# ruiminshen/yolo2-pytorch

Hardware: NVIDIA H100
Metric: 416x416 images/sec (higher is better)
Workload: dtype f16

## Files before the change

include/yolo2_b200.h:

```cpp
#ifndef YOLO2_B200_H_
#define YOLO2_B200_H_

#ifdef __cplusplus
extern "C" {
#endif

typedef void* yb_stream_t;

#define YB_ERR_BAD_ARG (-1)
#define YB_ERR_UNSUPPORTED (-2)
#define YB_ERR_DRIVER (-3)

#define YB_OUT_F16_NHWC 0
#define YB_OUT_F32_NCHW 1
#define YB_CONV_A_TILED 1
#define YB_CONV_WIDE_N 2
#define YB_CONV_FORCE_BN(bn) ((bn) << 8)
#define YB_CONV_POOL2X2 16
#define YB_CONV_C32_IM2COL 32
#define YB_CONV_NO_STREAMK 8
#define YB_CONV_FORCE_STREAMK (1 << 30)
#define YB_CONV_NO_SMALLK (1 << 28)
#define YB_CONV_PLAIN_STORE (1 << 29)
#define YB_FILTER_THRESHOLD 0
#define YB_FILTER_FIX 1
#define YB_FILTER_NONE 2

int yb_version(void);
const char* yb_last_error(void);
int yb_debug_read(int out[4]);
int yb_conv_set_trace(void* dev_buf);

int yb_pack_weight_f16(const float* w_oihw, void* w_f16, int cout, int cin, int ksize, int mode, yb_stream_t stream);
int yb_bn_fold(const float* gamma, const float* beta, const float* running_mean, const float* running_var, float eps, float* scale,
               float* shift, int channels, yb_stream_t stream);

int yb_conv0_bn_leaky_pool_fwd(const float* x_nchw, const float* w_oihw, const float* scale, const float* shift, float slope,
                               void* y_nhwc_f16, int batch, int height, int width, int cout, yb_stream_t stream);
int yb_conv0_u8_bn_leaky_pool_fwd(const unsigned char* x_nhwc_u8, const float* w_oihw, const float* scale, const float* shift,
                                  float slope, void* y_nhwc_f16, int batch, int height, int width, int cout, yb_stream_t stream);
int yb_conv_bn_act_fwd(const void* x, const void* w, const float* scale, const float* shift, float slope, void* y, int batch,
                       int height, int width, int cin, int cout, int ksize, int x_ld, long long y_ld, int y_ch_off, int out_mode,
                       int flags, yb_stream_t stream);
int yb_conv_bn_act_stats_fwd(const void* x, const void* w, const float* scale, const float* shift, float slope, void* y, int batch,
                             int height, int width, int cin, int cout, int ksize, int x_ld, long long y_ld, int y_ch_off, int flags,
                             double* sums, yb_stream_t stream);
long long yb_conv_workspace_bytes(void);
int yb_conv_choice(int batch, int height, int width, int cin, int cout, int ksize, int out_mode, int flags, int with_workspace, int out[6]);
int yb_conv_bn_act_fwd_ws(const void* x, const void* w, const float* scale, const float* shift, float slope, void* y, int batch,
                          int height, int width, int cin, int cout, int ksize, int x_ld, long long y_ld, int y_ch_off, int out_mode,
                          int flags, void* workspace, long long workspace_bytes, yb_stream_t stream);
int yb_conv_bn_act_split_fwd(const void* x, const void* w_split, const float* scale, const float* shift, float slope, void* y, int batch,
// ... 140 lines not shown
```

yolo2-pytorch_b200/b200/ops.py:

```python
import ctypes

import torch

from . import lib as _l

OUT_F16_NHWC, OUT_F32_NCHW = 0, 1
CONV_A_TILED, CONV_WIDE_N = 1, 2
CONV_NO_STREAMK, CONV_FORCE_STREAMK, CONV_NO_SMALLK, CONV_PLAIN_STORE = 8, 1 << 30, 1 << 28, 1 << 29
CONV_POOL2X2, CONV_C32_IM2COL, CONV_C32_SWAP = 16, 32, 64
FILTER_THRESHOLD, FILTER_FIX, FILTER_NONE = 0, 1, 2


launch_count = 0


def _ck(rc, what):
    global launch_count
    _l.check(rc, what)
    launch_count += 1


def conv_force_bn(bn):
    return bn << 8


def conv_force_mt(mt):
    return mt << 20


def conv_force_pair(v):
    return v << 22


CONV_ALLOW_PAIR = 4


def _p(t):
    return None if t is None else ctypes.c_void_p(t.data_ptr())


def _s():
    return ctypes.c_void_p(torch.cuda.current_stream().cuda_stream)
# ... 57 lines not shown
def conv0_u8_bn_leaky_pool(x, w, scale, shift, slope, out=None):
    _req(x, torch.uint8, 'x'); _req(w, torch.float32, 'w'); _req(scale, torch.float32, 'scale'); _req(shift, torch.float32, 'shift')
    b, h, wd, c = x.shape
    if c != 3:
        raise ValueError('conv0 expects 3 input channels')
    cout = w.shape[0]
    if out is None:
        out = torch.empty(b, h // 2, wd // 2, cout, dtype=torch.float16, device=x.device)
    _req(out, torch.float16, 'out')
    _ck(_l.load().yb_conv0_u8_bn_leaky_pool_fwd(_p(x), _p(w), _p(scale), _p(shift), float(slope), _p(out), b, h, wd, cout, _s()),
        'yb_conv0_u8_bn_leaky_pool_fwd')
    return out


def _conv_common(fn_name, x, w, scale, shift, slope, out, batch, height, width, cin, cout, k, x_ld, y_ld, y_ch_off, out_mode, flags,
                 workspace=None):
    if workspace is not None and fn_name == 'yb_conv_bn_act_fwd':
        fn_name = 'yb_conv_bn_act_fwd_ws'
    fn = getattr(_l.load(), fn_name)
    args = [_p(x), _p(w), _p(scale), _p(shift), float(slope), _p(out), batch, height, width, cin, cout, k, x_ld, y_ld, y_ch_off, out_mode]
    if fn_name != 'yb_conv_ref_fwd':
        args.append(flags)
    if fn_name == 'yb_conv_bn_act_fwd_ws':
        _req(workspace, torch.uint8, 'workspace')
        args += [_p(workspace), workspace.numel()]
    args.append(_s())
    _ck(fn(*args), fn_name)


def conv_workspace(device='cuda'):
    return torch.zeros(int(_l.load().yb_conv_workspace_bytes()), dtype=torch.uint8, device=device)


CONV_KERNELS = ('conv_igemm_kernel', 'conv_wide_kernel', 'conv_c32_kernel')


def conv_choice(batch, height, width, cin, cout, k, out_mode=OUT_F16_NHWC, flags=0, workspace=True):
    out = (ctypes.c_int * 6)()
    _l.check(_l.load().yb_conv_choice(batch, height, width, cin, cout, k, out_mode, flags, int(bool(workspace)), ctypes.byref(out)),
             'yb_conv_choice')
    return dict(kernel=CONV_KERNELS[out[0]], bk=out[1], bn=out[2], rows=out[3], streamk=bool(out[4]), grid=out[5])


def conv_bn_act(x, w, scale, shift, slope, out=None, out_mode=OUT_F16_NHWC, y_ch_off=0, cin=None, flags=0, ref=False, workspace=None):
    _req(x, torch.float16, 'x'); _req(w, torch.float16, 'w'); _req(scale, torch.float32, 'scale'); _req(shift, torch.float32, 'shift')
    b, h, wd, x_ld = x.shape
    cout, k, _, wcin = w.shape
    cin = wcin if cin is None else cin
    if cin != wcin:
        raise ValueError('weight Cin %d != %d' % (wcin, cin))
    if out is None:
        oh, ow = (h // 2, wd // 2) if (flags & CONV_POOL2X2) else (h, wd)
        out = (torch.empty(b, oh, ow, cout, dtype=torch.float16, device=x.device) if out_mode == OUT_F16_NHWC
               else torch.empty(b, cout, h, wd, dtype=torch.float32, device=x.device))
    if out_mode == OUT_F16_NHWC:
        _req(out, torch.float16, 'out')
        y_ld = out.shape[-1]
    else:
        _req(out, torch.float32, 'out')
        y_ld = 0
    _conv_common('yb_conv_ref_fwd' if ref else 'yb_conv_bn_act_fwd', x, w, scale, shift, slope, out, b, h, wd, cin, cout, k, x_ld, y_ld,
                 y_ch_off, out_mode, flags, workspace=None if ref else workspace)
    return out


def conv1x1_preact(x, w, pre_scale, pre_shift, pre_relu, scale, shift, slope, out=None, out_mode=OUT_F16_NHWC, y_ch_off=0, cin=None, flags=0,
                   workspace=None):
# ... 216 lines not shown
```

yolo2-pytorch_b200/csrc/conv_igemm.cu:

```cuda
#include "yb_common.h"
#include "yb_ptx.cuh"
#include <stdlib.h>

namespace yb {

struct ConvParams {
  int m_total;
  int height, width;
  int cin, cout;
  int ksize, pad;
  int kb_per_tap;
  int num_kb;
  int m_tiles, n_tiles;
  int a_im2col;
  const float* scale;
  const float* shift;
  float slope;
  void* y;
  long long y_ld;
  int y_ch_off;
  int out_mode;
  int hw;
  int skip;
  int* dbg;
// ... 739 lines not shown
          for (int h = 0; h < 2; ++h) {
#pragma unroll
            for (int hh = 0; hh < 2; ++hh) {
              const int j = c2 * 8 + jj;
              float x0 = acc[h][4 * j + 2 * hh] * sc0 + sh0;
              float x1 = acc[h][4 * j + 2 * hh + 1] * sc1 + sh1;
              x0 = x0 > 0.f ? x0 : x0 * p.slope;
              x1 = x1 > 0.f ? x1 : x1 * p.slope;
              __half2 v = __floats2half2_rn(x0, x1);
              const int r = h * 64 + warp * 16 + (lane >> 2) + hh * 8;
              const uint32_t addr = stage_o + r * 128 + ((jj ^ (r & 7)) << 4) + 4 * (lane & 3);
              asm volatile("st.shared.b32 [%0], %1;" :: "r"(addr), "r"(*reinterpret_cast<uint32_t*>(&v)) : "memory");
            }
          }
        }
        fence_proxy_async_smem();
        asm volatile("bar.sync %0, 128;" :: "r"(2 + cw) : "memory");
        if (t == 0) {
#pragma unroll
          for (int g = 0; g < 4; ++g)
            if (m_base + 32 * g < p.m_total) tma_store_2d(&tmap_y, stage_o + g * 4096, n0 + c2 * 64, m_base + 32 * g);
          tma_store_commit();
        }
      }
    }
    if (sk_collect) {
      asm volatile("bar.sync 1, 256;" ::: "memory");
      for (int j = sk_lo + t + 128 * cw; j < static_cast<int>(blockIdx.x); j += 256) p.flags[j] = 0u;
    }
  }
  if (t == 0) tma_store_wait<0>();
}

struct C32Params {
  int batch, height, width, cout;
  int tiles_w, tiles_h, num_tiles;
  const float* scale;
  const float* shift;
  float slope;
  int pool;
  int swap_lbo;
  int skip;
  int* dbg;
  unsigned long long* trace;
  double* stats;
};

struct C32Cfg {
  static constexpr int TH = 16, TW = 8, HH = TH + 2, HW = TW + 2;
  static constexpr int kPlaneData = HH * HW * 16;
  static constexpr int kPlane = (kPlaneData + 127) / 128 * 128;
  static constexpr int kHalo = 4 * kPlane;
  static constexpr int kStages = 4;
  static constexpr int BN = 64;
  static constexpr int kBTap = BN * 32 * 2;
  static constexpr int kBBytes = 9 * kBTap;
  static constexpr int kOutBytes = 128 * 128;
  static constexpr int kGroups = 2;
  static constexpr int kAccBytes = BN * kAccPitch * 4;
  static constexpr int kEpiThreads = kGroups * 128;
  static constexpr int kThreads = 128 + 32 + kEpiThreads;
  static constexpr int kSmemBytes = 1024 + kBBytes + 2 * kGroups * kOutBytes + kStages * kHalo + kGroups * kAccBytes + 2 * BN * 4 + 256 + 2 * BN * 4 ;
  static_assert(kSmemBytes <= kSmemLimit, "c32: shared memory budget");
};

__global__ void __launch_bounds__(C32Cfg::kThreads, 1)
// ... 186 lines not shown
      asm volatile("bar.sync %0, 128;" :: "r"(1 + grp) : "memory");
      if (et == 0) { YB_TRACE(2, tr); ++tr; }
      if (writer) {
#pragma unroll
        for (int c = 0; c < 8; ++c) st_shared_v4(obuf + srow * 128 + ((c ^ (srow & 7)) << 4), pk[c]);
      }
      fence_proxy_async_smem();
      asm volatile("bar.sync %0, 128;" :: "r"(1 + grp) : "memory");
      if (gt == 0 && !(p.skip & 8)) {
        if (p.pool) tma_store_4d(&tmap_y, obuf, 0, tw * (Cfg::TW / 2), th * (Cfg::TH / 2), n);
        else tma_store_4d(&tmap_y, obuf, 0, tw * Cfg::TW, th * Cfg::TH, n);
        tma_store_commit();
      }
      if (et == 0) { YB_TRACE(2, tr); ++tr; }
    }
    if (gt == 0) tma_store_wait<0>();
    if (p.stats != nullptr) {
      asm volatile("bar.sync 8, %0;" :: "n"(Cfg::kEpiThreads) : "memory");
      for (int i = et; i < p.cout; i += Cfg::kEpiThreads) {
        atomicAdd(p.stats + i, static_cast<double>(ep_stats[i]));
        atomicAdd(p.stats + p.cout + i, static_cast<double>(ep_stats[BN + i]));
      }
    }
  }
}

constexpr long long kSkFlagBytes = 4096;
constexpr long long kSkSlotBytes = kWideRows * kWideBN * 4;
long long conv_workspace_bytes() { return kSkFlagBytes + kSkSlotBytes * sm_count(); }

constexpr int kKernelIgemm = 0;
constexpr int kKernelWide = 1;
constexpr int kKernelC32 = 2;
struct ConvChoice {
  int kernel, bk, bn, mt, streamk, grid;
};

static unsigned long long* g_conv_trace = nullptr;
void conv_set_trace(void* dev_ptr) { g_conv_trace = static_cast<unsigned long long*>(dev_ptr); }

typedef CUresult (*EncodeTiledFn)(CUtensorMap*, CUtensorMapDataType, cuuint32_t, void*, const cuuint64_t*, const cuuint64_t*,
                                  const cuuint32_t*, const cuuint32_t*, CUtensorMapInterleave, CUtensorMapSwizzle,
                                  CUtensorMapL2promotion, CUtensorMapFloatOOBfill);
typedef CUresult (*EncodeIm2colFn)(CUtensorMap*, CUtensorMapDataType, cuuint32_t, void*, const cuuint64_t*, const cuuint64_t*,
                                   const int*, const int*, cuuint32_t, cuuint32_t, const cuuint32_t*, CUtensorMapInterleave,
                                   CUtensorMapSwizzle, CUtensorMapL2promotion, CUtensorMapFloatOOBfill);

static int get_encoders(EncodeTiledFn* tiled, EncodeIm2colFn* im2col) {
  static EncodeTiledFn s_tiled = nullptr;
  static EncodeIm2colFn s_im2col = nullptr;
  if (s_tiled == nullptr || s_im2col == nullptr) {
    void* f0 = nullptr;
    void* f1 = nullptr;
    cudaDriverEntryPointQueryResult q0, q1;
    YB_CUDA(cudaGetDriverEntryPoint("cuTensorMapEncodeTiled", &f0, cudaEnableDefault, &q0));
    YB_CUDA(cudaGetDriverEntryPoint("cuTensorMapEncodeIm2col", &f1, cudaEnableDefault, &q1));
    if (f0 == nullptr || f1 == nullptr || q0 != cudaDriverEntryPointSuccess || q1 != cudaDriverEntryPointSuccess)
      return fail(YB_ERR_DRIVER, "cuTensorMapEncode* driver entry points unavailable");
    s_tiled = reinterpret_cast<EncodeTiledFn>(f0);
    s_im2col = reinterpret_cast<EncodeIm2colFn>(f1);
  }
  *tiled = s_tiled;
  *im2col = s_im2col;
  return 0;
}

int get_tensor_map_encoders(EncodeTiledFn* tiled, EncodeIm2colFn* im2col) { return get_encoders(tiled, im2col); }

// ... 31 lines not shown
  if (pre != nullptr) {
    YB_CUDA(cudaLaunchKernelEx(&cfg, conv_preact_kernel<BN, BK, MT>, ta, tb, ty, p, *pre));
    return check_launch("conv_preact_kernel");
  }
  YB_CUDA(cudaLaunchKernelEx(&cfg, conv_igemm_kernel<BN, BK, MT>, ta, tb, ty, p));
  return check_launch("conv_igemm_kernel");
}

template <int BK>
static int launch_wide(const CUtensorMap& ta, const CUtensorMap& tb, const CUtensorMap& ty, const ConvParams& p, int grid, cudaStream_t stream) {
  using Cfg = WideCfg<BK>;
  static bool attr_set = false;
  if (!attr_set) {
    YB_CUDA(cudaFuncSetAttribute(conv_wide_kernel<BK>, cudaFuncAttributeMaxDynamicSharedMemorySize, Cfg::kSmemBytes));
    attr_set = true;
  }
  cudaLaunchConfig_t cfg;
  memset(&cfg, 0, sizeof(cfg));
  cudaLaunchAttribute attr[1];
  int nattr = 0;
  static const int use_pdl = getenv("YB_PDL") ? atoi(getenv("YB_PDL")) : 0;
  if (use_pdl) {
    attr[nattr].id = cudaLaunchAttributeProgrammaticStreamSerialization;
    attr[nattr].val.programmaticStreamSerializationAllowed = 1;
    ++nattr;
  }
  cfg.gridDim = dim3(grid);
  cfg.blockDim = dim3(kWideThreads);
  cfg.dynamicSmemBytes = Cfg::kSmemBytes;
  cfg.stream = stream;
  cfg.attrs = attr; cfg.numAttrs = nattr;
  YB_CUDA(cudaLaunchKernelEx(&cfg, conv_wide_kernel<BK>, ta, tb, ty, p));
  return check_launch("conv_wide_kernel");
}

template <int BK>
static int dispatch_conv(int bn, int mt, int grid, const CUtensorMap& ta, const CUtensorMap& tb, const CUtensorMap& ty, const ConvParams& p,
                         const PreAct* pre, cudaStream_t stream) {
  if (mt == 2 && bn == 128) return launch_wide<BK>(ta, tb, ty, p, grid, stream);
  if (mt == 2) return launch_conv<64, BK, 2>(ta, tb, ty, p, pre, stream);
  if (bn == 64) return launch_conv<64, BK, 1>(ta, tb, ty, p, pre, stream);
  return launch_conv<128, BK, 1>(ta, tb, ty, p, pre, stream);
}

static int conv_c32_forward(const void* x, const void* w, const float* scale, const float* shift, float slope, void* y, int batch,
                            int height, int width, int cout, int x_ld, long long y_ld, int y_ch_off, int pool, int flags, double* stats,
                            cudaStream_t stream) {
  using Cfg = C32Cfg;
  EncodeTiledFn enc_tiled;
  EncodeIm2colFn enc_im2col;
  int rc = get_encoders(&enc_tiled, &enc_im2col);
  if (rc) return rc;
  YB_REQUIRE(!pool || (height % 2 == 0 && width % 2 == 0), "conv: fused 2x2 max-pool needs even H and W");
  C32Params p;
  p.batch = batch; p.height = height; p.width = width; p.cout = cout;
  p.tiles_w = (width + Cfg::TW - 1) / Cfg::TW;
  p.tiles_h = (height + Cfg::TH - 1) / Cfg::TH;
  const long long nt = static_cast<long long>(batch) * p.tiles_w * p.tiles_h;
  YB_REQUIRE(nt < (1ll << 31), "conv: too many tiles");
  p.num_tiles = static_cast<int>(nt);
  p.scale = scale; p.shift = shift; p.slope = slope;
  p.pool = pool;
  p.swap_lbo = (flags >> 6) & 1;
  p.skip = (flags >> 24) & 0xF;
  p.dbg = debug_word_device();
  p.trace = g_conv_trace;
// ... 43 lines not shown

constexpr double kKbNsIm2col = 240.0;
constexpr double kKbNsTiled = 100.0;
constexpr double kFeedBytesPerNs = 130.0;
constexpr double kEpiNsPerOut = 0.15;
constexpr double kWideEpiNsPerOut = 0.08;
constexpr double kSkNs = 16000.0;
constexpr double kSkNsWide = 9000.0;
int conv_choose(int batch, int height, int width, int cin, int cout, int ksize, int a_channels, int out_mode, int flags, bool workspace_ok,
                bool stats, bool lo, bool pre, ConvChoice* out) {
  ConvChoice c;
  memset(&c, 0, sizeof(c));
  const int sms = sm_count();
  const bool split = a_channels != cin || lo;
  if (!split && cin == 32 && ksize == 3 && cout <= 64 && out_mode == 0 && ((flags >> 28) & 1) == 0 && ((flags >> 5) & 1) == 0 && ((flags >> 8) & 0xFFFF) == 0) {
    const long long tiles = static_cast<long long>(batch) * ((width + C32Cfg::TW - 1) / C32Cfg::TW) * ((height + C32Cfg::TH - 1) / C32Cfg::TH);
    c.kernel = kKernelC32; c.bk = 32; c.bn = C32Cfg::BN; c.mt = 1;
    c.grid = static_cast<int>(tiles < sms ? tiles : sms);
    *out = c;
    return 0;
  }
  if ((flags >> 4) & 1) return fail(YB_ERR_UNSUPPORTED, "conv: YB_CONV_POOL2X2 is only implemented for the Cin = 32 3x3 layer");
  const int bk = (cin % 64 == 0 && a_channels % 64 == 0) ? 64 : 32;
  const bool sk_possible = !stats && workspace_ok && (flags & 8) == 0;
  const bool sk_force = sk_possible && ((flags >> 30) & 1);
  const bool wide_ok = out_mode == 0 && !lo && !stats && !pre && ((flags >> 24) & 0xF) == 0 && ((flags >> 29) & 1) == 0;
  const int force_bn = (flags >> 8) & 0x3FF;
  const int force_mt = (flags >> 20) & 0x3;
  const int force_pair = (flags >> 22) & 0x3;
  YB_REQUIRE(force_pair != 2, "conv: CTA-pair tiles need two-CTA tensor-core instructions, which sm_90 does not have");
  YB_REQUIRE(!force_bn || ((force_bn == 64 || force_bn == 128) && (force_mt != 2 || force_bn == 64 || wide_ok)),
             "conv: BLOCK_N=%d x %d M-subtiles is not a tile shape of this launch (64 x 1, 128 x 1, 64 x 2; 128 x 2 for fp16 NHWC "
             "outputs without residual or statistics)", force_bn, force_mt ? force_mt : 1);
  const long long m_total = static_cast<long long>(batch) * height * width;
  const int num_kb = ksize * ksize * (cin / bk);
  double best = 1e300;
  for (int cbn = 64; cbn <= 128; cbn *= 2) {
    if (force_bn && cbn != force_bn) continue;
    if (!force_bn && cbn > 64 && cbn / 2 >= cout) continue;
    for (int cmt = 1; cmt <= 2; ++cmt) {
      if (force_mt && cmt != force_mt) continue;
      const bool cwide = cmt * cbn > 128;
      if (cwide && !wide_ok) continue;
      const int rows_tile = BM * cmt;
      const double tiles = static_cast<double>((m_total + rows_tile - 1) / rows_tile) * ((cout + cbn - 1) / cbn);
      const double rounds = static_cast<double>((static_cast<long long>(tiles) + sms - 1) / sms);
      const double kb_ns = (ksize == 3 ? kKbNsIm2col : kKbNsTiled) + (cmt * BM + cbn) * bk * 2.0 / kFeedBytesPerNs;
      const double main_ns = num_kb * kb_ns;
      const double outs = static_cast<double>(rows_tile) * cbn;
      const double tile_ns = cwide ? main_ns + outs * kWideEpiNsPerOut : (main_ns > outs * kEpiNsPerOut ? main_ns : outs * kEpiNsPerOut);
      double t = rounds * tile_ns;
      int csk = 0;
      if (sk_possible) {
        const double units = tiles * num_kb;
        const double per_cta = static_cast<double>((static_cast<long long>(units) + sms - 1) / sms);
        const double tsk = per_cta * kb_ns + (cwide ? kSkNsWide : kSkNs);
        const bool ok = per_cta >= 4.0 && num_kb >= 2;
        const bool idle = tiles <= sms / 2;
        if (ok && (sk_force || (idle && tsk < 0.93 * t))) { t = tsk; csk = 1; }
      }
      if (sk_force && !csk) continue;
      if (t < best * 0.9999 || (t <= best * 1.0001 && cbn > c.bn)) { best = t; c.bn = cbn; c.mt = cmt; c.streamk = csk; }
    }
  }
  if (c.bn == 0) { c.bn = force_bn ? force_bn : 128; c.mt = force_mt ? force_mt : 1; c.streamk = 0; }
  YB_REQUIRE((c.bn == 64 || c.bn == 128) && (c.mt == 1 || c.mt == 2) && (c.mt * c.bn <= 128 || wide_ok), "conv: tile %d x %d", c.bn, c.mt);
  c.kernel = c.mt * c.bn > 128 ? kKernelWide : kKernelIgemm;
  c.bk = bk;
  const long long tiles = ((m_total + BM * c.mt - 1) / (BM * c.mt)) * ((cout + c.bn - 1) / c.bn);
  c.grid = c.streamk ? sms : static_cast<int>(tiles < sms ? tiles : sms);
  *out = c;
  return 0;
}

int conv_choice(int batch, int height, int width, int cin, int cout, int ksize, int out_mode, int flags, int with_workspace, int* out) {
  YB_REQUIRE(out != nullptr && batch > 0 && height > 0 && width > 0 && cin % 32 == 0 && cout > 0 && (ksize == 1 || ksize == 3),
             "conv_choice: bad shape");
  ConvChoice c;
  const int rc = conv_choose(batch, height, width, cin, cout, ksize, cin, out_mode, flags, with_workspace != 0, false, false, false, &c);
  if (rc) return rc;
  out[0] = c.kernel; out[1] = c.bk; out[2] = c.bn; out[3] = c.kernel == kKernelC32 ? C32Cfg::TH * C32Cfg::TW : BM * c.mt;
  out[4] = c.streamk; out[5] = c.grid;
  return 0;
}

int conv_igemm_forward(const void* x, const void* w, const float* scale, const float* shift, float slope, void* y, int batch,
                       int height, int width, int cin, int cout, int ksize, int x_ld, long long y_ld, int y_ch_off, int out_mode,
                       int flags, void* workspace, long long workspace_bytes, double* stats, int a_channels, int lo_ch_off,
                       const float* pre_scale, const float* pre_shift, int pre_relu, cudaStream_t stream) {
  YB_REQUIRE(x && w && scale && shift && y, "conv: null pointer");
  const bool pre = pre_scale != nullptr;
  if (pre) {
    YB_REQUIRE(pre_shift != nullptr && (pre_relu == 0 || pre_relu == 1), "conv_preact: pre_shift must be given, pre_relu 0 or 1");
    YB_REQUIRE(ksize == 1, "conv_preact: k=%d, the pre-activation form is 1x1 only", ksize);
    YB_REQUIRE(a_channels <= 0 || a_channels == cin, "conv_preact: split-precision operands are not supported");
    YB_REQUIRE(lo_ch_off < 0 && stats == nullptr, "conv_preact: no residual output and no fused statistics");
    YB_REQUIRE(cin <= kPreMaxCh, "conv_preact: Cin=%d exceeds the %d-channel pre-activation table", cin, kPreMaxCh);
  }
  const PreAct pre_act{pre_scale, pre_shift, pre_relu};
  if (a_channels <= 0) a_channels = cin;
  YB_REQUIRE(a_channels <= cin && a_channels % 32 == 0 && cin - a_channels <= a_channels, "conv: a_channels=%d does not fit cin=%d", a_channels, cin);
  YB_REQUIRE(lo_ch_off < 0 || (out_mode == 0 && stats == nullptr && lo_ch_off % 8 == 0 && lo_ch_off >= y_ch_off + cout && lo_ch_off + cout <= y_ld),
             "conv: lo_ch_off=%d (needs fp16 NHWC output with room for a second Cout-wide slice)", lo_ch_off);
  YB_REQUIRE(stats == nullptr || out_mode == 0, "conv: fused statistics need the fp16 NHWC output");
  YB_REQUIRE(ksize == 1 || ksize == 3, "conv: ksize %d unsupported (1 or 3)", ksize);
  YB_REQUIRE(batch > 0 && height > 0 && width > 0, "conv: bad shape");
  YB_REQUIRE(cin % 32 == 0, "conv: Cin=%d must be a multiple of 32 (layer 0 uses yb_conv0_*)", cin);
  YB_REQUIRE(x_ld >= a_channels && x_ld % 8 == 0, "conv: x_ld=%d", x_ld);
  YB_REQUIRE((reinterpret_cast<uintptr_t>(x) & 15) == 0 && (reinterpret_cast<uintptr_t>(w) & 15) == 0, "conv: x/w must be 16B aligned");
  YB_REQUIRE(out_mode == 0 || out_mode == 1, "conv: out_mode");
  if (out_mode == 0) {
    YB_REQUIRE(cout % 8 == 0 && y_ld % 8 == 0 && y_ch_off % 8 == 0 && (reinterpret_cast<uintptr_t>(y) & 15) == 0,
               "conv: fp16 NHWC output needs Cout, y_ld, y_ch_off multiples of 8 and a 16B aligned pointer");
  }
  const long long m_total_ll = static_cast<long long>(batch) * height * width;
  YB_REQUIRE(m_total_ll < (1ll << 31) - kWideRows, "conv: too many pixels");
  const bool ws_ok = workspace != nullptr && workspace_bytes >= conv_workspace_bytes() && (reinterpret_cast<uintptr_t>(workspace) & 255) == 0;
  ConvChoice ch;
  int rc = conv_choose(batch, height, width, cin, cout, ksize, a_channels, out_mode, flags, ws_ok, stats != nullptr, lo_ch_off >= 0, pre, &ch);
  if (rc) return rc;
  YB_REQUIRE(!pre || ch.kernel == kKernelIgemm, "conv_preact: no pre-activation form of kernel %d", ch.kernel);
  if (ch.kernel == kKernelC32)
    return conv_c32_forward(x, w, scale, shift, slope, y, batch, height, width, cout, x_ld, y_ld, y_ch_off, (flags >> 4) & 1, flags, stats, stream);
  const int bk = ch.bk, bn = ch.bn, mt = ch.mt, streamk = ch.streamk;
  static const int k1x1_im2col = getenv("YB_CONV_1X1_IM2COL") ? atoi(getenv("YB_CONV_1X1_IM2COL")) : 0;
  const int a_im2col = (ksize == 3) ? 1 : ((k1x1_im2col && !(flags & 1) && !pre) ? 1 : 0);

  EncodeTiledFn enc_tiled;
  EncodeIm2colFn enc_im2col;
  rc = get_encoders(&enc_tiled, &enc_im2col);
  if (rc) return rc;

  ConvParams p;
  p.m_total = static_cast<int>(m_total_ll);
  p.height = height; p.width = width; p.cin = cin; p.cout = cout; p.ksize = ksize; p.pad = (ksize - 1) / 2;
  p.kb_per_tap = cin / bk;
  p.num_kb = ksize * ksize * p.kb_per_tap;
  const int rows_tile = BM * mt;
  p.m_tiles = (p.m_total + rows_tile - 1) / rows_tile;
  p.n_tiles = (cout + bn - 1) / bn;
  p.a_im2col = a_im2col;
  p.scale = scale; p.shift = shift; p.slope = slope;
  p.y = y; p.y_ld = y_ld; p.y_ch_off = y_ch_off; p.out_mode = out_mode;
  p.hw = height * width;
  p.dbg = debug_word_device();
  p.trace = g_conv_trace;
  p.skip = (flags >> 24) & 0xF;
  p.streamk = streamk;
  p.stats = stats;
  p.tma_store = 0;
  p.a_wrap = a_channels;
  p.lo_off = lo_ch_off >= 0 ? static_cast<long long>(lo_ch_off - y_ch_off) : 0;
  p.sk_base = 0; p.sk_rem = 0; p.ws = nullptr; p.flags = nullptr;
  if (streamk) {
    const long long units = static_cast<long long>(p.m_tiles) * p.n_tiles * p.num_kb;
    YB_REQUIRE(units < (1ll << 31), "conv: stream-K unit count overflows");
    p.sk_base = static_cast<int>(units / sm_count());
    p.sk_rem = static_cast<int>(units % sm_count());
    p.flags = static_cast<unsigned*>(workspace);
    p.ws = reinterpret_cast<float*>(static_cast<char*>(workspace) + kSkFlagBytes);
  }

  const CUtensorMapSwizzle swz = (bk == 64) ? CU_TENSOR_MAP_SWIZZLE_128B : CU_TENSOR_MAP_SWIZZLE_64B;
  alignas(64) CUtensorMap ta, tb;
  CUresult cr;
  const int a_rows = BM * mt;
  if (a_im2col) {
    const cuuint64_t dims[4] = {static_cast<cuuint64_t>(a_channels), static_cast<cuuint64_t>(width), static_cast<cuuint64_t>(height),
                                static_cast<cuuint64_t>(batch)};
    const cuuint64_t strides[3] = {static_cast<cuuint64_t>(x_ld) * 2, static_cast<cuuint64_t>(x_ld) * 2 * width,
                                   static_cast<cuuint64_t>(x_ld) * 2 * width * height};
    const int lower[2] = {-p.pad, -p.pad};
    const int upper[2] = {p.pad - (ksize - 1), p.pad - (ksize - 1)};
    const cuuint32_t estr[4] = {1, 1, 1, 1};
    cr = enc_im2col(&ta, CU_TENSOR_MAP_DATA_TYPE_FLOAT16, 4, const_cast<void*>(x), dims, strides, lower, upper,
                    static_cast<cuuint32_t>(bk), static_cast<cuuint32_t>(a_rows), estr, CU_TENSOR_MAP_INTERLEAVE_NONE, swz, CU_TENSOR_MAP_L2_PROMOTION_L2_128B,
                    CU_TENSOR_MAP_FLOAT_OOB_FILL_NONE);
    if (cr != CUDA_SUCCESS) return fail(YB_ERR_DRIVER, "cuTensorMapEncodeIm2col failed (%d)", static_cast<int>(cr));
    int drv = 0;
    cudaDriverGetVersion(&drv);
    const unsigned long long span_bytes = static_cast<unsigned long long>(x_ld) * 2ull * width * height * batch;
    if (drv <= 13010 && span_bytes < 131072ull) reinterpret_cast<uint64_t*>(&ta)[1] &= ~(1ull << 21);
  } else {
    const cuuint64_t dims[2] = {static_cast<cuuint64_t>(a_channels), static_cast<cuuint64_t>(p.m_total)};
    const cuuint64_t strides[1] = {static_cast<cuuint64_t>(x_ld) * 2};
    const cuuint32_t box[2] = {static_cast<cuuint32_t>(bk), static_cast<cuuint32_t>(a_rows)};
    const cuuint32_t estr[2] = {1, 1};
    cr = enc_tiled(&ta, CU_TENSOR_MAP_DATA_TYPE_FLOAT16, 2, const_cast<void*>(x), dims, strides, box, estr,
                   CU_TENSOR_MAP_INTERLEAVE_NONE, swz, CU_TENSOR_MAP_L2_PROMOTION_L2_128B, CU_TENSOR_MAP_FLOAT_OOB_FILL_NONE);
    if (cr != CUDA_SUCCESS) return fail(YB_ERR_DRIVER, "cuTensorMapEncodeTiled(A) failed (%d)", static_cast<int>(cr));
  }
  {
    const cuuint64_t k_total = static_cast<cuuint64_t>(ksize) * ksize * cin;
    const cuuint64_t dims[2] = {k_total, static_cast<cuuint64_t>(cout)};
    const cuuint64_t strides[1] = {k_total * 2};
    const cuuint32_t box[2] = {static_cast<cuuint32_t>(bk), static_cast<cuuint32_t>(bn)};
    const cuuint32_t estr[2] = {1, 1};
    cr = enc_tiled(&tb, CU_TENSOR_MAP_DATA_TYPE_FLOAT16, 2, const_cast<void*>(w), dims, strides, box, estr,
                   CU_TENSOR_MAP_INTERLEAVE_NONE, swz, CU_TENSOR_MAP_L2_PROMOTION_L2_256B, CU_TENSOR_MAP_FLOAT_OOB_FILL_NONE);
    if (cr != CUDA_SUCCESS) return fail(YB_ERR_DRIVER, "cuTensorMapEncodeTiled(W) failed (%d)", static_cast<int>(cr));
  }

  alignas(64) CUtensorMap ty;
  memset(&ty, 0, sizeof(ty));
  p.tma_store = (out_mode == 0 && lo_ch_off < 0 && ((flags >> 29) & 1) == 0) ? 1 : 0;
  if (p.tma_store) {
    const cuuint64_t dims[2] = {static_cast<cuuint64_t>(cout), static_cast<cuuint64_t>(p.m_total)};
    const cuuint64_t strides[1] = {static_cast<cuuint64_t>(y_ld) * 2};
    const cuuint32_t box[2] = {64, 32};
    const cuuint32_t estr[2] = {1, 1};
    cr = enc_tiled(&ty, CU_TENSOR_MAP_DATA_TYPE_FLOAT16, 2, static_cast<__half*>(y) + y_ch_off, dims, strides, box, estr,
                   CU_TENSOR_MAP_INTERLEAVE_NONE, CU_TENSOR_MAP_SWIZZLE_128B, CU_TENSOR_MAP_L2_PROMOTION_NONE, CU_TENSOR_MAP_FLOAT_OOB_FILL_NONE);
    if (cr != CUDA_SUCCESS) return fail(YB_ERR_DRIVER, "cuTensorMapEncodeTiled(Y) failed (%d)", static_cast<int>(cr));
  }
  if (bk == 64) return dispatch_conv<64>(bn, mt, ch.grid, ta, tb, ty, p, pre ? &pre_act : nullptr, stream);
  return dispatch_conv<32>(bn, mt, ch.grid, ta, tb, ty, p, pre ? &pre_act : nullptr, stream);
}

__global__ void conv_ref_kernel(const __half* __restrict__ x, const __half* __restrict__ w, ConvParams p, int x_ld) {
  const long long idx = static_cast<long long>(blockIdx.x) * blockDim.x + threadIdx.x;
  const long long total = static_cast<long long>(p.m_total) * p.cout;
  if (idx >= total) return;
  const int co = static_cast<int>(idx % p.cout);
  const int row = static_cast<int>(idx / p.cout);
  const int img = row / p.hw;
  const int pix = row - img * p.hw;
  const int h = pix / p.width;
  const int wq = pix - h * p.width;
  float acc = 0.f;
  for (int r = 0; r < p.ksize; ++r) {
    const int hi = h + r - p.pad;
    if (hi < 0 || hi >= p.height) continue;
    for (int s = 0; s < p.ksize; ++s) {
      const int wi = wq + s - p.pad;
      if (wi < 0 || wi >= p.width) continue;
      const __half* xp = x + (static_cast<long long>(img) * p.hw + static_cast<long long>(hi) * p.width + wi) * x_ld;
      const __half* wp = w + (static_cast<long long>(co) * p.ksize * p.ksize + r * p.ksize + s) * p.cin;
      for (int c = 0; c < p.cin; ++c) acc += __half2float(xp[c]) * __half2float(wp[c]);
    }
  }
  float v = acc * p.scale[co] + p.shift[co];
  v = v > 0.f ? v : v * p.slope;
  if (p.out_mode == 0) {
    reinterpret_cast<__half*>(p.y)[static_cast<long long>(row) * p.y_ld + p.y_ch_off + co] = __float2half_rn(v);
  } else {
    reinterpret_cast<float*>(p.y)[(static_cast<long long>(img) * p.cout + co) * p.hw + pix] = v;
  }
// ... 20 lines not shown
```

Baseline: 18150.

## Add 192x256 tall-tile warp-specialized conv kernel with three consumer warpgroups

Adds a new persistent conv kernel that uses a 192-row by 256-column tile. One producer warp issues TMA loads and three consumer warpgroups each issue 64x256 wgmma, followed by a fused BN+leaky epilogue with TMA stores. The tile chooser now models this tile and selects it when cout exceeds 128 and the estimated time beats the existing wide/igemm choices without stream-K. The larger tile is meant to raise operand reuse per byte loaded from shared memory and L2, in exchange for fewer pipeline stages, higher register pressure and coarser tiles that can cause wave quantization.

```diff
diff --git a/include/yolo2_b200.h b/include/yolo2_b200.h
--- a/include/yolo2_b200.h
+++ b/include/yolo2_b200.h
@@ -18,6 +18,7 @@
 #define YB_CONV_FORCE_BN(bn) ((bn) << 8)
 #define YB_CONV_POOL2X2 16
 #define YB_CONV_C32_IM2COL 32
+#define YB_CONV_FORCE_TALL 128
 #define YB_CONV_NO_STREAMK 8
 #define YB_CONV_FORCE_STREAMK (1 << 30)
 #define YB_CONV_NO_SMALLK (1 << 28)
diff --git a/yolo2-pytorch_b200/b200/ops.py b/yolo2-pytorch_b200/b200/ops.py
--- a/yolo2-pytorch_b200/b200/ops.py
+++ b/yolo2-pytorch_b200/b200/ops.py
@@ -8,6 +8,7 @@
 CONV_A_TILED, CONV_WIDE_N = 1, 2
 CONV_NO_STREAMK, CONV_FORCE_STREAMK, CONV_NO_SMALLK, CONV_PLAIN_STORE = 8, 1 << 30, 1 << 28, 1 << 29
 CONV_POOL2X2, CONV_C32_IM2COL, CONV_C32_SWAP = 16, 32, 64
+CONV_FORCE_TALL = 128
 FILTER_THRESHOLD, FILTER_FIX, FILTER_NONE = 0, 1, 2
 
 
@@ -131,7 +132,7 @@
     return torch.zeros(int(_l.load().yb_conv_workspace_bytes()), dtype=torch.uint8, device=device)
 
 
-CONV_KERNELS = ('conv_igemm_kernel', 'conv_wide_kernel', 'conv_c32_kernel')
+CONV_KERNELS = ('conv_igemm_kernel', 'conv_wide_kernel', 'conv_c32_kernel', 'conv_tall_kernel')
 
 
 def conv_choice(batch, height, width, cin, cout, k, out_mode=OUT_F16_NHWC, flags=0, workspace=True):
diff --git a/yolo2-pytorch_b200/csrc/conv_igemm.cu b/yolo2-pytorch_b200/csrc/conv_igemm.cu
--- a/yolo2-pytorch_b200/csrc/conv_igemm.cu
+++ b/yolo2-pytorch_b200/csrc/conv_igemm.cu
@@ -795,6 +795,162 @@
   if (t == 0) tma_store_wait<0>();
 }
 
+constexpr int kTallThreads = 512;
+constexpr int kTallRows = 192;
+constexpr int kTallBN = 256;
+
+template <int BK>
+struct TallCfg {
+  static constexpr int kSwizzle = BK * 2;
+  static constexpr int kABytes = kTallRows * BK * 2;
+  static constexpr int kBBytes = kTallBN * BK * 2;
+  static constexpr int kStageBytes = kABytes + kBBytes;
+  static constexpr int kOutBytes = 64 * 128;
+  static constexpr int kFixedBytes = 3 * kOutBytes + 1024  + 256 ;
+  static constexpr int kStages = ((kSmemLimit - kFixedBytes) / kStageBytes) > 8 ? 8 : ((kSmemLimit - kFixedBytes) / kStageBytes);
+  static constexpr int kSmemBytes = kStages * kStageBytes + kFixedBytes;
+  static_assert(kStages >= 3, "shared memory budget");
+  static_assert(kABytes % 1024 == 0 && kBBytes % 1024 == 0, "stages must keep the swizzle atoms aligned");
+};
+
+template <int BK>
+__global__ void __launch_bounds__(kTallThreads, 1)
+conv_tall_kernel(const __grid_constant__ CUtensorMap tmap_a, const __grid_constant__ CUtensorMap tmap_b,
+                 const __grid_constant__ CUtensorMap tmap_y, const ConvParams p) {
+  using Cfg = TallCfg<BK>;
+  constexpr int kStages = Cfg::kStages;
+  extern __shared__ uint8_t smem_raw[];
+  const uint32_t smem_base = (smem_u32(smem_raw) + 1023u) & ~1023u;
+  const uint32_t smem_a = smem_base;
+  const uint32_t smem_b = smem_base + kStages * Cfg::kABytes;
+  const uint32_t smem_o = smem_base + kStages * Cfg::kStageBytes;
+  const uint32_t bar_full = smem_o + 3 * Cfg::kOutBytes;
+  const uint32_t bar_empty = bar_full + 8 * kStages;
+  const int num_tiles = p.m_tiles * p.n_tiles;
+
+  if (threadIdx.x == 0) {
+    for (int i = 0; i < kStages; ++i) {
+      mbar_init(bar_full + 8 * i, 1);
+      mbar_init(bar_empty + 8 * i, 12);
+    }
+    fence_mbar_init();
+    fence_proxy_async_smem();
+    tma_prefetch_desc(&tmap_a);
+    tma_prefetch_desc(&tmap_b);
+    tma_prefetch_desc(&tmap_y);
+  }
+  __syncthreads();
+  pdl_trigger();
+  pdl_wait();
+
+  if (threadIdx.x < 128) {
+    setmaxnreg_dec<32>();
+    if (threadIdx.x == 0) {
+      int stage = 0;
+      uint32_t phase = 0;
+      for (int tile = blockIdx.x; tile < num_tiles; tile += gridDim.x) {
+        const int n_tile = tile % p.n_tiles;
+        const int m_cta = (tile / p.n_tiles) * kTallRows;
+        const int img = m_cta / p.hw;
+        const int rem = m_cta - img * p.hw;
+        const int h0 = rem / p.width;
+        const int w0 = rem - h0 * p.width;
+        for (int kb = 0; kb < p.num_kb; ++kb) {
+          const int tap = kb / p.kb_per_tap;
+          const int c0 = (kb - tap * p.kb_per_tap) * BK;
+          const int r = tap / p.ksize;
+          const int s = tap - r * p.ksize;
+          mbar_wait(bar_empty + 8 * stage, phase ^ 1, p.dbg, 0xC00 | stage);
+          const uint32_t full = bar_full + 8 * stage;
+          mbar_arrive_expect_tx(full, Cfg::kStageBytes);
+          const uint32_t dst = smem_a + stage * Cfg::kABytes;
+          if (p.a_im2col) tma_load_im2col_4d(dst, &tmap_a, full, c0, w0 - p.pad, h0 - p.pad, img, static_cast<uint16_t>(s), static_cast<uint16_t>(r));
+          else tma_load_2d(dst, &tmap_a, full, c0, m_cta);
+          tma_load_2d(smem_b + stage * Cfg::kBBytes, &tmap_b, full, tap * p.cin + c0, n_tile * kTallBN);
+          if (++stage == kStages) { stage = 0; phase ^= 1; }
+        }
+      }
+      for (int i = 0; i < kStages; ++i) {
+        mbar_wait(bar_empty + 8 * stage, phase ^ 1, p.dbg, 0xC00 | stage);
+        if (++stage == kStages) { stage = 0; phase ^= 1; }
+      }
+    }
+    return;
+  }
+  setmaxnreg_inc<160>();
+  const int cw = (threadIdx.x >> 7) - 1;
+  const int t = threadIdx.x & 127;
+  const int warp = t >> 5;
+  const int lane = t & 31;
+  const uint32_t stage_o = smem_o + cw * Cfg::kOutBytes;
+  float acc[2][64];
+  int stage = 0;
+  uint32_t phase = 0;
+  for (int tile = blockIdx.x; tile < num_tiles; tile += gridDim.x) {
+    int prev = -1;
+    for (int kb = 0; kb < p.num_kb; ++kb) {
+      while (!mbar_try_wait(bar_full + 8 * stage, phase)) {}
+      const uint64_t adesc = make_kmajor_desc<Cfg::kSwizzle>(smem_a + stage * Cfg::kABytes + cw * 64 * Cfg::kSwizzle);
+      wgmma_fence();
+#pragma unroll
+      for (int k = 0; k < BK / UMMA_K; ++k)
+#pragma unroll
+        for (int nh = 0; nh < 2; ++nh) {
+          const uint64_t bdesc = make_kmajor_desc<Cfg::kSwizzle>(smem_b + stage * Cfg::kBBytes + nh * 128 * Cfg::kSwizzle);
+          wgmma_f16<128>(acc[nh], adesc + 2 * k, bdesc + 2 * k, (kb | k) != 0);
+        }
+      wgmma_commit();
+      wgmma_wait<1>();
+      if (prev >= 0) { __syncwarp(); if (lane == 0) mbar_arrive(bar_empty + 8 * prev); }
+      prev = stage;
+      if (++stage == kStages) { stage = 0; phase ^= 1; }
+    }
+    wgmma_wait<0>();
+    fence_regs(acc[0]);
+    fence_regs(acc[1]);
+    __syncwarp();
+    if (lane == 0) mbar_arrive(bar_empty + 8 * prev);
+
+    const int n0 = (tile % p.n_tiles) * kTallBN;
+    const int m_base = (tile / p.n_tiles) * kTallRows + cw * 64;
+#pragma unroll
+    for (int c4 = 0; c4 < kTallBN / 64; ++c4) {
+      if (n0 + c4 * 64 < p.cout) {
+        if (t == 0) tma_store_wait_read<0>();
+        asm volatile("bar.sync %0, 128;" :: "r"(2 + cw) : "memory");
+#pragma unroll
+        for (int jj = 0; jj < 8; ++jj) {
+          const int col = n0 + c4 * 64 + 8 * jj + 2 * (lane & 3);
+          const bool ok = col < p.cout;
+          const float sc0 = ok ? __ldg(p.scale + col) : 0.f, sc1 = ok ? __ldg(p.scale + col + 1) : 0.f;
+          const float sh0 = ok ? __ldg(p.shift + col) : 0.f, sh1 = ok ? __ldg(p.shift + col + 1) : 0.f;
+#pragma unroll
+          for (int hh = 0; hh < 2; ++hh) {
+            const int j = (c4 & 1) * 8 + jj;
+            float x0 = acc[c4 >> 1][4 * j + 2 * hh] * sc0 + sh0;
+            float x1 = acc[c4 >> 1][4 * j + 2 * hh + 1] * sc1 + sh1;
+            x0 = x0 > 0.f ? x0 : x0 * p.slope;
+            x1 = x1 > 0.f ? x1 : x1 * p.slope;
+            __half2 v = __floats2half2_rn(x0, x1);
+            const int r = warp * 16 + (lane >> 2) + hh * 8;
+            const uint32_t addr = stage_o + r * 128 + ((jj ^ (r & 7)) << 4) + 4 * (lane & 3);
+            asm volatile("st.shared.b32 [%0], %1;" :: "r"(addr), "r"(*reinterpret_cast<uint32_t*>(&v)) : "memory");
+          }
+        }
+        fence_proxy_async_smem();
+        asm volatile("bar.sync %0, 128;" :: "r"(2 + cw) : "memory");
+        if (t == 0) {
+#pragma unroll
+          for (int g = 0; g < 2; ++g)
+            if (m_base + 32 * g < p.m_total) tma_store_2d(&tmap_y, stage_o + g * 4096, n0 + c4 * 64, m_base + 32 * g);
+          tma_store_commit();
+        }
+      }
+    }
+  }
+  if (t == 0) tma_store_wait<0>();
+}
+
 struct C32Params {
   int batch, height, width, cout;
   int tiles_w, tiles_h, num_tiles;
@@ -1047,8 +1203,10 @@
 constexpr int kKernelIgemm = 0;
 constexpr int kKernelWide = 1;
 constexpr int kKernelC32 = 2;
+constexpr int kKernelTall = 3;
 struct ConvChoice {
   int kernel, bk, bn, mt, streamk, grid;
+  int rows;
 };
 
 static unsigned long long* g_conv_trace = nullptr;
@@ -1146,6 +1304,33 @@
   cfg.attrs = attr; cfg.numAttrs = nattr;
   YB_CUDA(cudaLaunchKernelEx(&cfg, conv_wide_kernel<BK>, ta, tb, ty, p));
   return check_launch("conv_wide_kernel");
+}
+
+template <int BK>
+static int launch_tall(const CUtensorMap& ta, const CUtensorMap& tb, const CUtensorMap& ty, const ConvParams& p, int grid, cudaStream_t stream) {
+  using Cfg = TallCfg<BK>;
+  static bool attr_set = false;
+  if (!attr_set) {
+    YB_CUDA(cudaFuncSetAttribute(conv_tall_kernel<BK>, cudaFuncAttributeMaxDynamicSharedMemorySize, Cfg::kSmemBytes));
+    attr_set = true;
+  }
+  cudaLaunchConfig_t cfg;
+  memset(&cfg, 0, sizeof(cfg));
+  cudaLaunchAttribute attr[1];
+  int nattr = 0;
+  static const int use_pdl = getenv("YB_PDL") ? atoi(getenv("YB_PDL")) : 0;
+  if (use_pdl) {
+    attr[nattr].id = cudaLaunchAttributeProgrammaticStreamSerialization;
+    attr[nattr].val.programmaticStreamSerializationAllowed = 1;
+    ++nattr;
+  }
+  cfg.gridDim = dim3(grid);
+  cfg.blockDim = dim3(kTallThreads);
+  cfg.dynamicSmemBytes = Cfg::kSmemBytes;
+  cfg.stream = stream;
+  cfg.attrs = attr; cfg.numAttrs = nattr;
+  YB_CUDA(cudaLaunchKernelEx(&cfg, conv_tall_kernel<BK>, ta, tb, ty, p));
+  return check_launch("conv_tall_kernel");
 }
 
 template <int BK>
@@ -1255,10 +1440,14 @@
   YB_REQUIRE(!force_bn || ((force_bn == 64 || force_bn == 128) && (force_mt != 2 || force_bn == 64 || wide_ok)),
              "conv: BLOCK_N=%d x %d M-subtiles is not a tile shape of this launch (64 x 1, 128 x 1, 64 x 2; 128 x 2 for fp16 NHWC "
              "outputs without residual or statistics)", force_bn, force_mt ? force_mt : 1);
+  const bool force_tall = (flags >> 7) & 1;
+  const bool tall_ok = wide_ok && !split && !force_bn && !force_mt && !sk_force;
+  YB_REQUIRE(!force_tall || tall_ok, "conv: the 192 x 256 tile needs an fp16 NHWC output without residual, statistics, split operands, "
+             "stream-K or another forced tile shape");
   const long long m_total = static_cast<long long>(batch) * height * width;
   const int num_kb = ksize * ksize * (cin / bk);
   double best = 1e300;
-  for (int cbn = 64; cbn <= 128; cbn *= 2) {
+  for (int cbn = 64; cbn <= 128 && !force_tall; cbn *= 2) {
     if (force_bn && cbn != force_bn) continue;
     if (!force_bn && cbn > 64 && cbn / 2 >= cout) continue;
     for (int cmt = 1; cmt <= 2; ++cmt) {
@@ -1286,11 +1475,21 @@
       if (t < best * 0.9999 || (t <= best * 1.0001 && cbn > c.bn)) { best = t; c.bn = cbn; c.mt = cmt; c.streamk = csk; }
     }
   }
+  bool tall = false;
+  if (force_tall || (tall_ok && cout > kTallBN / 2)) {
+    const double tiles = static_cast<double>((m_total + kTallRows - 1) / kTallRows) * ((cout + kTallBN - 1) / kTallBN);
+    const double rounds = static_cast<double>((static_cast<long long>(tiles) + sms - 1) / sms);
+    const double wide_kb_ns = (ksize == 3 ? kKbNsIm2col : kKbNsTiled) + (kWideRows + kWideBN) * bk * 2.0 / kFeedBytesPerNs;
+    const double kb_ns = wide_kb_ns * (static_cast<double>(kTallRows) * kTallBN) / (kWideRows * kWideBN);
+    const double t = rounds * (num_kb * kb_ns + static_cast<double>(kTallRows) * kTallBN * kWideEpiNsPerOut);
+    if (force_tall || (!c.streamk && t < best * 0.97)) { best = t; tall = true; c.bn = kTallBN; c.mt = 0; c.streamk = 0; }
+  }
   if (c.bn == 0) { c.bn = force_bn ? force_bn : 128; c.mt = force_mt ? force_mt : 1; c.streamk = 0; }
-  YB_REQUIRE((c.bn == 64 || c.bn == 128) && (c.mt == 1 || c.mt == 2) && (c.mt * c.bn <= 128 || wide_ok), "conv: tile %d x %d", c.bn, c.mt);
-  c.kernel = c.mt * c.bn > 128 ? kKernelWide : kKernelIgemm;
+  YB_REQUIRE(tall || ((c.bn == 64 || c.bn == 128) && (c.mt == 1 || c.mt == 2) && (c.mt * c.bn <= 128 || wide_ok)), "conv: tile %d x %d", c.bn, c.mt);
+  c.kernel = tall ? kKernelTall : c.mt * c.bn > 128 ? kKernelWide : kKernelIgemm;
   c.bk = bk;
-  const long long tiles = ((m_total + BM * c.mt - 1) / (BM * c.mt)) * ((cout + c.bn - 1) / c.bn);
+  c.rows = tall ? kTallRows : BM * c.mt;
+  const long long tiles = ((m_total + c.rows - 1) / c.rows) * ((cout + c.bn - 1) / c.bn);
   c.grid = c.streamk ? sms : static_cast<int>(tiles < sms ? tiles : sms);
   *out = c;
   return 0;
@@ -1302,7 +1501,7 @@
   ConvChoice c;
   const int rc = conv_choose(batch, height, width, cin, cout, ksize, cin, out_mode, flags, with_workspace != 0, false, false, false, &c);
   if (rc) return rc;
-  out[0] = c.kernel; out[1] = c.bk; out[2] = c.bn; out[3] = c.kernel == kKernelC32 ? C32Cfg::TH * C32Cfg::TW : BM * c.mt;
+  out[0] = c.kernel; out[1] = c.bk; out[2] = c.bn; out[3] = c.kernel == kKernelC32 ? C32Cfg::TH * C32Cfg::TW : c.rows;
   out[4] = c.streamk; out[5] = c.grid;
   return 0;
 }
@@ -1359,7 +1558,7 @@
   p.height = height; p.width = width; p.cin = cin; p.cout = cout; p.ksize = ksize; p.pad = (ksize - 1) / 2;
   p.kb_per_tap = cin / bk;
   p.num_kb = ksize * ksize * p.kb_per_tap;
-  const int rows_tile = BM * mt;
+  const int rows_tile = ch.rows;
   p.m_tiles = (p.m_total + rows_tile - 1) / rows_tile;
   p.n_tiles = (cout + bn - 1) / bn;
   p.a_im2col = a_im2col;
@@ -1387,7 +1586,7 @@
   const CUtensorMapSwizzle swz = (bk == 64) ? CU_TENSOR_MAP_SWIZZLE_128B : CU_TENSOR_MAP_SWIZZLE_64B;
   alignas(64) CUtensorMap ta, tb;
   CUresult cr;
-  const int a_rows = BM * mt;
+  const int a_rows = rows_tile;
   if (a_im2col) {
     const cuuint64_t dims[4] = {static_cast<cuuint64_t>(a_channels), static_cast<cuuint64_t>(width), static_cast<cuuint64_t>(height),
                                 static_cast<cuuint64_t>(batch)};
@@ -1436,6 +1635,7 @@
                    CU_TENSOR_MAP_INTERLEAVE_NONE, CU_TENSOR_MAP_SWIZZLE_128B, CU_TENSOR_MAP_L2_PROMOTION_NONE, CU_TENSOR_MAP_FLOAT_OOB_FILL_NONE);
     if (cr != CUDA_SUCCESS) return fail(YB_ERR_DRIVER, "cuTensorMapEncodeTiled(Y) failed (%d)", static_cast<int>(cr));
   }
+  if (ch.kernel == kKernelTall) return bk == 64 ? launch_tall<64>(ta, tb, ty, p, ch.grid, stream) : launch_tall<32>(ta, tb, ty, p, ch.grid, stream);
   if (bk == 64) return dispatch_conv<64>(bn, mt, ch.grid, ta, tb, ty, p, pre ? &pre_act : nullptr, stream);
   return dispatch_conv<32>(bn, mt, ch.grid, ta, tb, ty, p, pre ? &pre_act : nullptr, stream);
 }
```

After: 18220, median of 6. No clear change (+0.4%).
